# LukasHedegaard/continual-skeletons

Measured on AMD Instinct MI355X. Metric: clips/sec (ST-GCN clip forward, NTU-60 shape; CoST-GCN online step reported under costgcn_online), higher is better.
Workload: dtype f32

## Files before the change

### continual-skeletons_amd/csrc/tcn_wino.hip

```cpp
#include "mfma_core.h"
#include "tcn_params.h"

namespace {

constexpr int WMT = 64;
constexpr int WNT = 128;
constexpr int WTAPS = 12;

template <int VT>
constexpr int wino_ldb() { return ((2 * ((WNT + VT - 2) / VT) + 10) * VT + 3) / 4 * 4; }

struct WStage12x64 {
    unsigned goff0, loff0, gstride;
    f32x4 v[6];
    __device__ __forceinline__ void setup(int Cpad, int Mpad, int tid) {
        goff0 = (unsigned)(((tid >> 7) * Cpad + ((tid >> 4) & 7)) * Mpad + (tid & 15) * 4);
        loff0 = (unsigned)(tid * 4);
        gstride = (unsigned)(2 * Cpad * Mpad);
    }
    __device__ __forceinline__ void issue_slot(int u, const float *__restrict__ chunk_base) {
        v[u] = *reinterpret_cast<const f32x4 *>(chunk_base + (size_t)u * gstride + goff0);
    }
    __device__ __forceinline__ void issue(const float *__restrict__ chunk_base) {
#pragma unroll
        for (int u = 0; u < 6; ++u) issue_slot(u, chunk_base);
    }
    __device__ __forceinline__ void commit(float *__restrict__ Wl) const {
#pragma unroll
        for (int u = 0; u < 6; ++u) *reinterpret_cast<f32x4 *>(Wl + u * (NTHREADS * 4) + loff0) = v[u];
    }
};

template <int VT, int G>
__device__ __forceinline__ void wino_group(const float *__restrict__ Wl, const float *__restrict__ Bl, int off, int l31, int kh,
                                           f32x16 (&acc)[4][2]) {
    constexpr int LDB = wino_ldb<VT>();
    const float *br = Bl + kh * LDB + off + 3 * G * VT;
    const float *wr = Wl + 4 * G * (KC * WMT) + kh * WMT + l31;
#pragma unroll
    for (int s = 0; s < KC / 2; ++s) {
        const float d0 = br[2 * s * LDB], d1 = br[2 * s * LDB + VT], d2 = br[2 * s * LDB + 2 * VT], d3 = br[2 * s * LDB + 3 * VT];
        const float b[4] = {d0 - d2, d1 + d2, d2 - d1, d1 - d3};
#pragma unroll
        for (int i = 0; i < 4; ++i) {
            const float a0 = wr[i * (KC * WMT) + 2 * s * WMT], a1 = wr[i * (KC * WMT) + 2 * s * WMT + 32];
            acc[i][0] = __builtin_amdgcn_mfma_f32_32x32x2f32(a0, b[i], acc[i][0], 0, 0, 0);
            acc[i][1] = __builtin_amdgcn_mfma_f32_32x32x2f32(a1, b[i], acc[i][1], 0, 0, 0);
        }
    }
}

template <int VT, bool RES>
__device__ __forceinline__ void wino_epilogue(const TcnParams &p, const f32x16 (&acc)[4][2], int m0, int q0, int qend, int seg,
                                              int wave, int l31, int kh, int jc, int vc) {
    const int T = p.Tout, TV = T * VT;
    const bool qv = q0 + wave * 32 + l31 < qend;
    const bool odd_ok = 2 * jc + 1 < T;
    const unsigned p0 = (unsigned)(2 * jc * VT + vc);
    const unsigned b0 = 4u * (4u * (unsigned)kh * (unsigned)TV + p0);
    const unsigned b1 = odd_ok ? b0 + 4u * VT : b0;
    const unsigned kh16 = 16u * (unsigned)kh;
    const float *rseg = RES ? p.xres + (int64_t)seg * p.Cout * TV : nullptr;
    float *oseg = p.out + (int64_t)seg * p.Cout * TV;
#pragma unroll
    for (int mi = 0; mi < 2; ++mi) {
        const int rb = m0 + mi * 32;
        float o0[16], o1[16];
#pragma unroll
        for (int g = 0; g < 16; ++g) {
            const int row = rb + (g & 3) + 8 * (g >> 2);
            const float bias = ld_lane(p.bias + row, kh16);
            const float m1 = acc[1][mi][g], m2 = acc[2][mi][g];
            float v0 = acc[0][mi][g] + m1 + m2 + bias;
            float v1 = m1 - m2 - acc[3][mi][g] + bias;
            if (RES) {
                const float *rrow = rseg + (int64_t)row * TV;
                v0 += ld_lane(rrow, b0);
                v1 += ld_lane(rrow, b1);
            }
            if (p.relu) { v0 = relu_nan(v0); v1 = relu_nan(v1); }
            o0[g] = v0;
            o1[g] = v1;
        }
        if (qv) {
#pragma unroll
            for (int g = 0; g < 16; ++g) {
                float *orow = oseg + (int64_t)(rb + (g & 3) + 8 * (g >> 2)) * TV;
                st_lane(orow, b0, o0[g]);
                if (odd_ok) st_lane(orow, b1, o1[g]);
            }
        }
    }
}

}

template <int VT, bool RES = true>
__global__ __launch_bounds__(NTHREADS, 2) void tcn_stage_wino_kernel(const TcnParams p) {
    constexpr int LDB = wino_ldb<VT>();
    constexpr int NJ = (LDB + 63) / 64;
    extern __shared__ __attribute__((aligned(16))) float smem[];
    float *Wl = smem;
    float *Bl = smem + WTAPS * KC * WMT;

    const int tid = threadIdx.x, lane = tid & 63, wave = __builtin_amdgcn_readfirstlane(tid >> 6);
    const int l31 = lane & 31, kh = lane >> 5;
    const unsigned wid = xcd_contiguous_id(blockIdx.x, gridDim.x);
    const int m0 = (int)(wid % p.mtiles) * WMT, q0 = (int)((wid / p.mtiles) % p.qtiles) * WNT;
    const int seg = (int)(wid / (p.mtiles * p.qtiles));
    const int T = p.Tout, TV = T * VT, QP = p.nt;
    const int qend = min(q0 + WNT, QP);
    const int ja = div_magic(q0, p.vmagic), jb = div_magic(qend - 1, p.vmagic);

    const int qc = min(q0 + wave * 32 + l31, qend - 1);
    const int jc = div_magic(qc, p.vmagic), vc = qc - jc * VT;
    const int off = 2 * (jc - ja) * VT + vc;

    f32x16 acc[4][2];
#pragma unroll
    for (int i = 0; i < 4; ++i)
#pragma unroll
        for (int mi = 0; mi < 2; ++mi)
#pragma unroll
            for (int g = 0; g < 16; ++g) acc[i][mi][g] = 0.f;

    {
        const int fa = 2 * ja - 4;
        const int span = (2 * (jb - ja) + 10) * VT;
        const int64_t cs = (int64_t)TV;
        const float *seg_base = p.y + (int64_t)seg * p.C * cs;
        const float *wbase = p.w + m0;
        WStage12x64 ws;
        ws.setup(p.Cpad, p.Mpad, tid);
        auto kloop = [&](auto &bx) {
            ws.issue(wbase);
            bx.issue(seg_base, p.C, cs, 0, wave);
            for (int c0 = 0; c0 + KC < p.Cpad; c0 += KC) {
                __syncthreads();
                ws.commit(Wl);
                bx.commit(Bl, LDB, wave);
                __syncthreads();
                const float *wnext = wbase + (size_t)(c0 + KC) * p.Mpad;
                const int cn = c0 + KC;
                ws.issue_slot(0, wnext);
                ws.issue_slot(1, wnext);
                bx.template issue_third<0>(seg_base, p.C, cs, cn, wave);
                __builtin_amdgcn_s_setprio(1);
                wino_group<VT, 0>(Wl, Bl, off, l31, kh, acc);
                __builtin_amdgcn_s_setprio(0);
                ws.issue_slot(2, wnext);
                ws.issue_slot(3, wnext);
                bx.template issue_third<1>(seg_base, p.C, cs, cn, wave);
                __builtin_amdgcn_s_setprio(1);
                wino_group<VT, 1>(Wl, Bl, off, l31, kh, acc);
                __builtin_amdgcn_s_setprio(0);
                ws.issue_slot(4, wnext);
                ws.issue_slot(5, wnext);
                bx.template issue_third<2>(seg_base, p.C, cs, cn, wave);
                __builtin_amdgcn_s_setprio(1);
                wino_group<VT, 2>(Wl, Bl, off, l31, kh, acc);
                __builtin_amdgcn_s_setprio(0);
            }
            __syncthreads();
            ws.commit(Wl);
            bx.commit(Bl, LDB, wave);
            __syncthreads();
            wino_group<VT, 0>(Wl, Bl, off, l31, kh, acc);
            wino_group<VT, 1>(Wl, Bl, off, l31, kh, acc);
            wino_group<VT, 2>(Wl, Bl, off, l31, kh, acc);
        };
        const bool interior = fa >= 0 && fa * VT + 4 * ((span + 3) / 4) <= TV;
        if (interior) {
            BStage4<(NJ + 3) / 4> b4;
            b4.setup(fa * VT, span, lane);
            kloop(b4);
        } else {
            BStage<NJ> bs;
            bs.setup(fa * VT, span, TV, lane);
            kloop(bs);
        }
    }

    wino_epilogue<VT, RES>(p, acc, m0, q0, qend, seg, wave, l31, kh, jc, vc);
}

namespace {

constexpr int W2TAPS = 13;

template <int VT>
constexpr int wino2_ldb() { return ((4 * ((WNT + VT - 2) / VT) + 11) * VT + 3) / 4 * 4; }

struct WStage13x64 {
    unsigned goff0, loff0, gstride, u6;
    f32x4 v[7];
    __device__ __forceinline__ void setup(int Cpad, int Mpad, int tid) {
        goff0 = (unsigned)(((tid >> 7) * Cpad + ((tid >> 4) & 7)) * Mpad + (tid & 15) * 4);
        loff0 = (unsigned)(tid * 4);
        gstride = (unsigned)(2 * Cpad * Mpad);
        u6 = tid >= 128 ? 5u : 6u;
    }
    __device__ __forceinline__ void issue_slot(int u, const float *__restrict__ chunk_base) {
        if (u < 6) v[u] = *reinterpret_cast<const f32x4 *>(chunk_base + (size_t)u * gstride + goff0);
        else v[6] = *reinterpret_cast<const f32x4 *>(chunk_base + (size_t)u6 * gstride + goff0);
    }
    __device__ __forceinline__ void issue(const float *__restrict__ chunk_base) {
#pragma unroll
        for (int u = 0; u < 7; ++u) issue_slot(u, chunk_base);
    }
    __device__ __forceinline__ void commit(float *__restrict__ Wl) const {
#pragma unroll
        for (int u = 0; u < 6; ++u) *reinterpret_cast<f32x4 *>(Wl + u * (NTHREADS * 4) + loff0) = v[u];
        *reinterpret_cast<f32x4 *>(Wl + u6 * (NTHREADS * 4) + loff0) = v[6];
    }
};

struct WStageRes64 {
    unsigned goff0, loff0;
    f32x4 v;
    __device__ __forceinline__ void setup(int Mpad, int tid) {
        goff0 = (unsigned)(((tid >> 4) & 7) * Mpad + (tid & 15) * 4);
        loff0 = (unsigned)((tid & 127) * 4);
    }
    __device__ __forceinline__ void issue(const float *__restrict__ chunk_base) {
        v = *reinterpret_cast<const f32x4 *>(chunk_base + goff0);
    }
    __device__ __forceinline__ void commit(float *__restrict__ Wl) const { *reinterpret_cast<f32x4 *>(Wl + loff0) = v; }
};

template <int VT, int ROW0, int F, int NP>
__device__ __forceinline__ void wino2_group(const float *__restrict__ Wl, const float *__restrict__ Bl, int off, int l31, int kh,
                                            f32x16 (&acc)[4][2]) {
    constexpr int LDB = wino2_ldb<VT>();
    const float *br = Bl + kh * LDB + off + F * VT;
    const float *wr = Wl + ROW0 * (KC * WMT) + kh * WMT + l31;
#pragma unroll
    for (int s = 0; s < KC / 2; ++s) {
        const float d0 = br[2 * s * LDB], d1 = br[2 * s * LDB + 2 * VT], d2 = br[2 * s * LDB + 4 * VT];
        const float d3 = NP == 4 ? br[2 * s * LDB + 6 * VT] : 0.f;
        const float b[4] = {d0 - d2, d1 + d2, d2 - d1, d1 - d3};
#pragma unroll
        for (int i = 0; i < NP; ++i) {
            const float a0 = wr[i * (KC * WMT) + 2 * s * WMT], a1 = wr[i * (KC * WMT) + 2 * s * WMT + 32];
            acc[i][0] = __builtin_amdgcn_mfma_f32_32x32x2f32(a0, b[i], acc[i][0], 0, 0, 0);
            acc[i][1] = __builtin_amdgcn_mfma_f32_32x32x2f32(a1, b[i], acc[i][1], 0, 0, 0);
        }
    }
}

template <int VT>
__device__ __forceinline__ void wino2_res_chunk(const float *__restrict__ Wl, const float *__restrict__ Bl, int off, int l31, int kh,
                                                f32x16 (&acc)[4][2]) {
    constexpr int LDB = wino2_ldb<VT>();
    const float *br = Bl + kh * LDB + off;
    const float *wr = Wl + kh * WMT + l31;
#pragma unroll
    for (int s = 0; s < KC / 2; ++s) {
        const float d0 = br[2 * s * LDB], d1 = br[2 * s * LDB + 2 * VT];
        const float a0 = wr[2 * s * WMT], a1 = wr[2 * s * WMT + 32];
        const float b0 = d0 - d1;
        acc[0][0] = __builtin_amdgcn_mfma_f32_32x32x2f32(a0, b0, acc[0][0], 0, 0, 0);
        acc[0][1] = __builtin_amdgcn_mfma_f32_32x32x2f32(a1, b0, acc[0][1], 0, 0, 0);
        acc[1][0] = __builtin_amdgcn_mfma_f32_32x32x2f32(a0, d1, acc[1][0], 0, 0, 0);
        acc[1][1] = __builtin_amdgcn_mfma_f32_32x32x2f32(a1, d1, acc[1][1], 0, 0, 0);
    }
}

}

template <int VT, bool RESCONV>
__global__ __launch_bounds__(NTHREADS, 2) void tcn_stage_wino_s2_kernel(const TcnParams p) {
    constexpr int LDB = wino2_ldb<VT>();
    constexpr int NJ = (LDB + 63) / 64;
    constexpr int NJR = ((4 * ((WNT + VT - 2) / VT) + 3) * VT + 63) / 64;
    extern __shared__ __attribute__((aligned(16))) float smem[];
    float *Wl = smem;
    float *Bl = smem + W2TAPS * KC * WMT;

    const int tid = threadIdx.x, lane = tid & 63, wave = __builtin_amdgcn_readfirstlane(tid >> 6);
    const int l31 = lane & 31, kh = lane >> 5;
    const unsigned wid = xcd_contiguous_id(blockIdx.x, gridDim.x);
    const int m0 = (int)(wid % p.mtiles) * WMT, q0 = (int)((wid / p.mtiles) % p.qtiles) * WNT;
    const int seg = (int)(wid / (p.mtiles * p.qtiles));
    const int TVin = p.Tin * VT, QP = p.nt;
    const int qend = min(q0 + WNT, QP);
    const int ja = div_magic(q0, p.vmagic), jb = div_magic(qend - 1, p.vmagic);

    const int qc = min(q0 + wave * 32 + l31, qend - 1);
    const int jc = div_magic(qc, p.vmagic), vc = qc - jc * VT;
    const int off = 4 * (jc - ja) * VT + vc;

    f32x16 acc[4][2];
#pragma unroll
    for (int i = 0; i < 4; ++i)
#pragma unroll
        for (int mi = 0; mi < 2; ++mi)
#pragma unroll
            for (int g = 0; g < 16; ++g) acc[i][mi][g] = 0.f;

    {
        const int fa = 4 * ja - 4;
        const int span = (4 * (jb - ja) + 11) * VT;
        const int64_t cs = (int64_t)TVin;
        const float *seg_base = p.y + (int64_t)seg * p.C * cs;
        const float *wbase = p.w + m0;
        WStage13x64 ws;
        ws.setup(p.Cpad, p.Mpad, tid);
        auto kloop = [&](auto &bx) {
            ws.issue(wbase);
            bx.issue(seg_base, p.C, cs, 0, wave);
            for (int c0 = 0; c0 + KC < p.Cpad; c0 += KC) {
                __syncthreads();
                ws.commit(Wl);
                bx.commit(Bl, LDB, wave);
                __syncthreads();
                const float *wnext = wbase + (size_t)(c0 + KC) * p.Mpad;
                const int cn = c0 + KC;
                ws.issue_slot(0, wnext);
                ws.issue_slot(1, wnext);
                bx.template issue_third<0>(seg_base, p.C, cs, cn, wave);
                __builtin_amdgcn_s_setprio(1);
                wino2_group<VT, 0, 0, 4>(Wl, Bl, off, l31, kh, acc);
                __builtin_amdgcn_s_setprio(0);
                ws.issue_slot(2, wnext);
                ws.issue_slot(3, wnext);
                bx.template issue_third<1>(seg_base, p.C, cs, cn, wave);
                __builtin_amdgcn_s_setprio(1);
                wino2_group<VT, 4, 6, 3>(Wl, Bl, off, l31, kh, acc);
                __builtin_amdgcn_s_setprio(0);
                ws.issue_slot(4, wnext);
                ws.issue_slot(5, wnext);
                bx.template issue_third<2>(seg_base, p.C, cs, cn, wave);
                __builtin_amdgcn_s_setprio(1);
                wino2_group<VT, 7, 1, 3>(Wl, Bl, off, l31, kh, acc);
                __builtin_amdgcn_s_setprio(0);
                ws.issue_slot(6, wnext);
                __builtin_amdgcn_s_setprio(1);
                wino2_group<VT, 10, 5, 3>(Wl, Bl, off, l31, kh, acc);
                __builtin_amdgcn_s_setprio(0);
            }
            __syncthreads();
            ws.commit(Wl);
            bx.commit(Bl, LDB, wave);
            __syncthreads();
            wino2_group<VT, 0, 0, 4>(Wl, Bl, off, l31, kh, acc);
            wino2_group<VT, 4, 6, 3>(Wl, Bl, off, l31, kh, acc);
            wino2_group<VT, 7, 1, 3>(Wl, Bl, off, l31, kh, acc);
            wino2_group<VT, 10, 5, 3>(Wl, Bl, off, l31, kh, acc);
        };
        const bool interior = fa >= 0 && fa * VT + 4 * ((span + 3) / 4) <= TVin;
        if (interior) {
            BStage4<(NJ + 3) / 4> b4;
            b4.setup(fa * VT, span, lane);
            kloop(b4);
        } else {
            BStage<NJ> bs;
            bs.setup(fa * VT, span, TVin, lane);
            kloop(bs);
        }
    }

    if (RESCONV) {
        const int span = (4 * (jb - ja) + 3) * VT;
        const int64_t cs = (int64_t)p.Tres * VT;
        const float *seg_base = p.xres + (int64_t)seg * p.Cres * cs;
        const float *wbase = p.wres + m0;
        const int cend = (p.Cres + KC - 1) / KC * KC;
        WStageRes64 wr;
        wr.setup(p.Mpad, tid);
        BStage<NJR> bs;
        bs.setup(4 * ja * VT, span, p.Tres * VT, lane);
        wr.issue(wbase);
        bs.issue(seg_base, p.Cres, cs, 0, wave);
        for (int c0 = 0; c0 + KC < cend; c0 += KC) {
            __syncthreads();
            wr.commit(Wl);
            bs.commit(Bl, LDB, wave);
            __syncthreads();
            wr.issue(wbase + (size_t)(c0 + KC) * p.Mpad);
            bs.issue(seg_base, p.Cres, cs, c0 + KC, wave);
            wino2_res_chunk<VT>(Wl, Bl, off, l31, kh, acc);
        }
        __syncthreads();
        wr.commit(Wl);
        bs.commit(Bl, LDB, wave);
        __syncthreads();
        wino2_res_chunk<VT>(Wl, Bl, off, l31, kh, acc);
    }

    wino_epilogue<VT, false>(p, acc, m0, q0, qend, seg, wave, l31, kh, jc, vc);
}

static int tcn_stage_wino_launch(const float *y, const float *w_wino, const float *x_res, const float *bias, float *out, int n_seg,
                                 int c, int c_out, int t_in, int V, int k, int stride, int pad, int res_mode, int c_res, int t_res,
                                 int res_off, int relu, void *stream, bool res_none = false) {
    if (!w_wino || !y || !bias || !out) return -2;
    if (k != 9 || stride != 1 || pad != 4) return -2;
    if (res_none ? res_mode != CSK_RES_NONE : (res_mode != CSK_RES_IDENTITY || res_off != 0 || !x_res || c_res != c_out || t_res != t_in))
        return -2;
    if ((V != 25 && V != 18) || c_out % WMT != 0 || c < 1 || n_seg < 1 || t_in < 1) return -2;
    if ((int64_t)t_in * V >= (1 << 26)) return -2;
    if (csk_diag_flag("CSK_TCN_WINO")) return -2;
    const int qp = (t_in + 1) / 2 * V;
    const int qtiles = (qp + WNT - 1) / WNT, mtiles = c_out / WMT;
    if ((int64_t)qtiles * mtiles * n_seg >= (1ll << 31)) return -2;
    TcnParams p = {};
    p.y = y; p.w = w_wino; p.xres = res_none ? nullptr : x_res; p.wres = nullptr; p.bias = bias; p.out = out;
    p.C = c; p.Cpad = round_up(c, CSK_CPAD); p.Cout = c_out; p.Mpad = round_up(c_out, CSK_MT);
    p.Tin = t_in; p.Tout = t_in; p.V = V; p.K = k; p.stride = 1; p.pad = pad;
    p.res_mode = res_mode; p.Cres = res_none ? 0 : c_res; p.CresPad = round_up(p.Cres, CSK_CPAD); p.Tres = res_none ? 0 : t_res;
    p.res_off = 0; p.relu = relu;
    p.vmagic = vmagic_of(V); p.mtiles = (unsigned)mtiles; p.qtiles = (unsigned)qtiles; p.nt = qp;
    void (*kern)(TcnParams) = res_none ? (V == 25 ? tcn_stage_wino_kernel<25, false> : tcn_stage_wino_kernel<18, false>)
                                       : (V == 25 ? tcn_stage_wino_kernel<25> : tcn_stage_wino_kernel<18>);
    const int ldb = V == 25 ? wino_ldb<25>() : wino_ldb<18>();
    p.ldb = ldb;
    const size_t lds = (size_t)(WTAPS * KC * WMT + KC * ldb) * sizeof(float);
    if (const int e = csk_ensure_lds((const void *)kern, lds)) return e;
    hipLaunchKernelGGL(kern, dim3((unsigned)(qtiles * mtiles * n_seg)), dim3(NTHREADS), lds, (hipStream_t)stream, p);
    return (int)hipGetLastError();
}

static int tcn_stage_wino_s2_launch(const float *y, const float *w_s2, const float *x_res, const float *w_res, const float *bias,
                                    float *out, int n_seg, int c, int c_out, int t_in, int V, int k, int stride, int pad,
                                    int res_mode, int c_res, int t_res, int res_off, int relu, void *stream) {
    if (!w_s2 || !y || !bias || !out) return -2;
    if (k != 9 || stride != 2 || pad != 4 || res_off != 0) return -2;
    const bool conv = res_mode == CSK_RES_CONV;
    if (!conv && res_mode != CSK_RES_NONE) return -2;
    if (conv && (!x_res || !w_res || c_res < 1 || t_res != t_in)) return -2;
    if ((V != 25 && V != 18) || c_out % WMT != 0 || c < 1 || n_seg < 1 || t_in < 1) return -2;
    if ((int64_t)t_in * V >= (1 << 26)) return -2;
    if (csk_diag_flag("CSK_TCN_WINO")) return -2;
    const int t_out = (t_in - 1) / 2 + 1;
    const int qp = (t_out + 1) / 2 * V;
    const int qtiles = (qp + WNT - 1) / WNT, mtiles = c_out / WMT;
    if ((int64_t)qtiles * mtiles * n_seg >= (1ll << 31)) return -2;
    TcnParams p = {};
    p.y = y; p.w = w_s2; p.xres = conv ? x_res : nullptr; p.wres = conv ? w_res : nullptr; p.bias = bias; p.out = out;
    p.C = c; p.Cpad = round_up(c, CSK_CPAD); p.Cout = c_out; p.Mpad = round_up(c_out, CSK_MT);
    p.Tin = t_in; p.Tout = t_out; p.V = V; p.K = k; p.stride = 2; p.pad = pad;
    p.res_mode = res_mode; p.Cres = conv ? c_res : 0; p.CresPad = round_up(p.Cres, CSK_CPAD); p.Tres = conv ? t_res : 0;
    p.res_off = 0; p.relu = relu;
    p.vmagic = vmagic_of(V); p.mtiles = (unsigned)mtiles; p.qtiles = (unsigned)qtiles; p.nt = qp;
    void (*kern)(TcnParams) = conv ? (V == 25 ? tcn_stage_wino_s2_kernel<25, true> : tcn_stage_wino_s2_kernel<18, true>)
                                   : (V == 25 ? tcn_stage_wino_s2_kernel<25, false> : tcn_stage_wino_s2_kernel<18, false>);
    const int ldb = V == 25 ? wino2_ldb<25>() : wino2_ldb<18>();
    p.ldb = ldb;
    const size_t lds = (size_t)(W2TAPS * KC * WMT + KC * ldb) * sizeof(float);
    if (const int e = csk_ensure_lds((const void *)kern, lds)) return e;
    hipLaunchKernelGGL(kern, dim3((unsigned)(qtiles * mtiles * n_seg)), dim3(NTHREADS), lds, (hipStream_t)stream, p);
    return (int)hipGetLastError();
}

extern "C" int csk_tcn_stage_wino_f32(const float *y, const float *w, const float *x_res, const float *w_res, const float *bias,
                                      float *out, int n_seg, int c, int c_out, int t_in, int V, int k, int stride, int pad,
                                      int res_mode, int c_res, int t_res, int res_off, int relu, const float *w_wino, void *stream) {
    const int rc = tcn_stage_wino_launch(y, w_wino, x_res, bias, out, n_seg, c, c_out, t_in, V, k, stride, pad, res_mode, c_res,
                                         t_res, res_off, relu, stream);
    if (rc != -2) return rc;
    return csk_tcn_stage_f32(y, w, x_res, w_res, bias, out, n_seg, c, c_out, t_in, V, k, stride, pad, res_mode, c_res, t_res,
                             res_off, relu, stream);
}

extern "C" int csk_tcn_stage_wino_ext_f32(const float *y, const float *w, const float *x_res, const float *w_res, const float *bias,
                                          float *out, int n_seg, int c, int c_out, int t_in, int V, int k, int stride, int pad,
                                          int res_mode, int c_res, int t_res, int res_off, int relu, const float *w_wino_ext,
                                          void *stream) {
    int rc = -2;
    if (stride == 1)
        rc = tcn_stage_wino_launch(y, w_wino_ext, nullptr, bias, out, n_seg, c, c_out, t_in, V, k, stride, pad, res_mode, c_res,
                                   t_res, res_off, relu, stream, true);
    else if (stride == 2)
        rc = tcn_stage_wino_s2_launch(y, w_wino_ext, x_res, w_res, bias, out, n_seg, c, c_out, t_in, V, k, stride, pad, res_mode,
                                      c_res, t_res, res_off, relu, stream);
    if (rc != -2) return rc;
    return csk_tcn_stage_f32(y, w, x_res, w_res, bias, out, n_seg, c, c_out, t_in, V, k, stride, pad, res_mode, c_res, t_res,
                             res_off, relu, stream);
}
```

Before: 4158.

## Add 128x64 Winograd TCN tile variant with 2x2 wave layout

Adds an MW=2 variant of the stride-1 and stride-2 Winograd temporal-conv kernels. Each block covers 128 output channels by 64 positions, with waves arranged 2x2 instead of 1x4, and new weight and input staging structs sized for the taller tile. A heuristic uses it by default for stride-2 stages, and for stride-1 stages when the narrower position tile wastes less padding. The aim is more reuse of the input B-tile across output channels and less tail waste on the position axis. The cost is a larger LDS weight footprint, fewer blocks in flight, and more template instantiations.

Result: faster. 4268 (median of 6 runs) (+2.7%).

```diff
diff --git a/continual-skeletons_amd/csrc/tcn_wino.hip b/continual-skeletons_amd/csrc/tcn_wino.hip
--- a/continual-skeletons_amd/csrc/tcn_wino.hip
+++ b/continual-skeletons_amd/csrc/tcn_wino.hip
@@ -1,3 +1,5 @@
+#include <type_traits>
+
 #include "mfma_core.h"
 #include "tcn_params.h"
 
@@ -7,8 +9,8 @@
 constexpr int WNT = 128;
 constexpr int WTAPS = 12;
 
-template <int VT>
-constexpr int wino_ldb() { return ((2 * ((WNT + VT - 2) / VT) + 10) * VT + 3) / 4 * 4; }
+template <int VT, int MW = 1>
+constexpr int wino_ldb() { return ((2 * ((WNT / MW + VT - 2) / VT) + 10) * VT + 3) / 4 * 4; }
 
 struct WStage12x64 {
     unsigned goff0, loff0, gstride;
@@ -25,25 +27,58 @@
 #pragma unroll
         for (int u = 0; u < 6; ++u) issue_slot(u, chunk_base);
     }
+    template <int G>
+    __device__ __forceinline__ void issue_part(const float *__restrict__ chunk_base) {
+        issue_slot(2 * G, chunk_base);
+        issue_slot(2 * G + 1, chunk_base);
+    }
     __device__ __forceinline__ void commit(float *__restrict__ Wl) const {
 #pragma unroll
         for (int u = 0; u < 6; ++u) *reinterpret_cast<f32x4 *>(Wl + u * (NTHREADS * 4) + loff0) = v[u];
     }
 };
 
-template <int VT, int G>
+template <int NT>
+struct WStageNx128 {
+    unsigned goff0, loff0, gstride;
+    f32x4 v[NT];
+    __device__ __forceinline__ void setup(int Cpad, int Mpad, int tid) {
+        goff0 = 4u * (unsigned)((tid >> 5) * Mpad + (tid & 31) * 4);
+        loff0 = (unsigned)(tid * 4);
+        gstride = (unsigned)(Cpad * Mpad);
+    }
+    __device__ __forceinline__ void issue_slot(int u, const float *__restrict__ chunk_base) {
+        v[u] = *reinterpret_cast<const f32x4 *>(reinterpret_cast<const char *>(chunk_base + (size_t)u * gstride) + goff0);
+    }
+    __device__ __forceinline__ void issue(const float *__restrict__ chunk_base) {
+#pragma unroll
+        for (int u = 0; u < NT; ++u) issue_slot(u, chunk_base);
+    }
+    template <int G>
+    __device__ __forceinline__ void issue_part(const float *__restrict__ chunk_base) {
+        constexpr int lo = NT == 13 ? (G == 0 ? 0 : 3 * G + 1) : 4 * G, hi = NT == 13 ? 3 * G + 4 : 4 * G + 4;
+#pragma unroll
+        for (int u = lo; u < hi; ++u) issue_slot(u, chunk_base);
+    }
+    __device__ __forceinline__ void commit(float *__restrict__ Wl) const {
+#pragma unroll
+        for (int u = 0; u < NT; ++u) *reinterpret_cast<f32x4 *>(Wl + u * (KC * 128) + loff0) = v[u];
+    }
+};
+
+template <int VT, int G, int MW>
 __device__ __forceinline__ void wino_group(const float *__restrict__ Wl, const float *__restrict__ Bl, int off, int l31, int kh,
                                            f32x16 (&acc)[4][2]) {
-    constexpr int LDB = wino_ldb<VT>();
+    constexpr int LDB = wino_ldb<VT, MW>(), MT = WMT * MW;
     const float *br = Bl + kh * LDB + off + 3 * G * VT;
-    const float *wr = Wl + 4 * G * (KC * WMT) + kh * WMT + l31;
+    const float *wr = Wl + 4 * G * (KC * MT) + kh * MT + l31;
 #pragma unroll
     for (int s = 0; s < KC / 2; ++s) {
         const float d0 = br[2 * s * LDB], d1 = br[2 * s * LDB + VT], d2 = br[2 * s * LDB + 2 * VT], d3 = br[2 * s * LDB + 3 * VT];
         const float b[4] = {d0 - d2, d1 + d2, d2 - d1, d1 - d3};
 #pragma unroll
         for (int i = 0; i < 4; ++i) {
-            const float a0 = wr[i * (KC * WMT) + 2 * s * WMT], a1 = wr[i * (KC * WMT) + 2 * s * WMT + 32];
+            const float a0 = wr[i * (KC * MT) + 2 * s * MT], a1 = wr[i * (KC * MT) + 2 * s * MT + 32];
             acc[i][0] = __builtin_amdgcn_mfma_f32_32x32x2f32(a0, b[i], acc[i][0], 0, 0, 0);
             acc[i][1] = __builtin_amdgcn_mfma_f32_32x32x2f32(a1, b[i], acc[i][1], 0, 0, 0);
         }
@@ -52,9 +87,9 @@
 
 template <int VT, bool RES>
 __device__ __forceinline__ void wino_epilogue(const TcnParams &p, const f32x16 (&acc)[4][2], int m0, int q0, int qend, int seg,
-                                              int wave, int l31, int kh, int jc, int vc) {
+                                              int wn, int l31, int kh, int jc, int vc) {
     const int T = p.Tout, TV = T * VT;
-    const bool qv = q0 + wave * 32 + l31 < qend;
+    const bool qv = q0 + wn * 32 + l31 < qend;
     const bool odd_ok = 2 * jc + 1 < T;
     const unsigned p0 = (unsigned)(2 * jc * VT + vc);
     const unsigned b0 = 4u * (4u * (unsigned)kh * (unsigned)TV + p0);
@@ -95,24 +130,25 @@
 
 }
 
-template <int VT, bool RES = true>
+template <int VT, bool RES = true, int MW = 1>
 __global__ __launch_bounds__(NTHREADS, 2) void tcn_stage_wino_kernel(const TcnParams p) {
-    constexpr int LDB = wino_ldb<VT>();
+    constexpr int LDB = wino_ldb<VT, MW>(), MT = WMT * MW, NT = WNT / MW;
     constexpr int NJ = (LDB + 63) / 64;
     extern __shared__ __attribute__((aligned(16))) float smem[];
     float *Wl = smem;
-    float *Bl = smem + WTAPS * KC * WMT;
+    float *Bl = smem + WTAPS * KC * MT;
 
     const int tid = threadIdx.x, lane = tid & 63, wave = __builtin_amdgcn_readfirstlane(tid >> 6);
     const int l31 = lane & 31, kh = lane >> 5;
+    const int wm = MW == 2 ? wave >> 1 : 0, wn = MW == 2 ? wave & 1 : wave;
     const unsigned wid = xcd_contiguous_id(blockIdx.x, gridDim.x);
-    const int m0 = (int)(wid % p.mtiles) * WMT, q0 = (int)((wid / p.mtiles) % p.qtiles) * WNT;
+    const int m0 = (int)(wid % p.mtiles) * MT, q0 = (int)((wid / p.mtiles) % p.qtiles) * NT;
     const int seg = (int)(wid / (p.mtiles * p.qtiles));
     const int T = p.Tout, TV = T * VT, QP = p.nt;
-    const int qend = min(q0 + WNT, QP);
+    const int qend = min(q0 + NT, QP);
     const int ja = div_magic(q0, p.vmagic), jb = div_magic(qend - 1, p.vmagic);
 
-    const int qc = min(q0 + wave * 32 + l31, qend - 1);
+    const int qc = min(q0 + wn * 32 + l31, qend - 1);
     const int jc = div_magic(qc, p.vmagic), vc = qc - jc * VT;
     const int off = 2 * (jc - ja) * VT + vc;
 
@@ -130,7 +166,8 @@
         const int64_t cs = (int64_t)TV;
         const float *seg_base = p.y + (int64_t)seg * p.C * cs;
         const float *wbase = p.w + m0;
-        WStage12x64 ws;
+        const float *Ww = Wl + wm * WMT;
+        std::conditional_t<MW == 2, WStageNx128<WTAPS>, WStage12x64> ws;
         ws.setup(p.Cpad, p.Mpad, tid);
         auto kloop = [&](auto &bx) {
             ws.issue(wbase);
@@ -142,32 +179,29 @@
                 __syncthreads();
                 const float *wnext = wbase + (size_t)(c0 + KC) * p.Mpad;
                 const int cn = c0 + KC;
-                ws.issue_slot(0, wnext);
-                ws.issue_slot(1, wnext);
+                ws.template issue_part<0>(wnext);
                 bx.template issue_third<0>(seg_base, p.C, cs, cn, wave);
                 __builtin_amdgcn_s_setprio(1);
-                wino_group<VT, 0>(Wl, Bl, off, l31, kh, acc);
+                wino_group<VT, 0, MW>(Ww, Bl, off, l31, kh, acc);
                 __builtin_amdgcn_s_setprio(0);
-                ws.issue_slot(2, wnext);
-                ws.issue_slot(3, wnext);
+                ws.template issue_part<1>(wnext);
                 bx.template issue_third<1>(seg_base, p.C, cs, cn, wave);
                 __builtin_amdgcn_s_setprio(1);
-                wino_group<VT, 1>(Wl, Bl, off, l31, kh, acc);
+                wino_group<VT, 1, MW>(Ww, Bl, off, l31, kh, acc);
                 __builtin_amdgcn_s_setprio(0);
-                ws.issue_slot(4, wnext);
-                ws.issue_slot(5, wnext);
+                ws.template issue_part<2>(wnext);
                 bx.template issue_third<2>(seg_base, p.C, cs, cn, wave);
                 __builtin_amdgcn_s_setprio(1);
-                wino_group<VT, 2>(Wl, Bl, off, l31, kh, acc);
+                wino_group<VT, 2, MW>(Ww, Bl, off, l31, kh, acc);
                 __builtin_amdgcn_s_setprio(0);
             }
             __syncthreads();
             ws.commit(Wl);
             bx.commit(Bl, LDB, wave);
             __syncthreads();
-            wino_group<VT, 0>(Wl, Bl, off, l31, kh, acc);
-            wino_group<VT, 1>(Wl, Bl, off, l31, kh, acc);
-            wino_group<VT, 2>(Wl, Bl, off, l31, kh, acc);
+            wino_group<VT, 0, MW>(Ww, Bl, off, l31, kh, acc);
+            wino_group<VT, 1, MW>(Ww, Bl, off, l31, kh, acc);
+            wino_group<VT, 2, MW>(Ww, Bl, off, l31, kh, acc);
         };
         const bool interior = fa >= 0 && fa * VT + 4 * ((span + 3) / 4) <= TV;
         if (interior) {
@@ -181,15 +215,15 @@
         }
     }
 
-    wino_epilogue<VT, RES>(p, acc, m0, q0, qend, seg, wave, l31, kh, jc, vc);
+    wino_epilogue<VT, RES>(p, acc, m0 + wm * WMT, q0, qend, seg, wn, l31, kh, jc, vc);
 }
 
 namespace {
 
 constexpr int W2TAPS = 13;
 
-template <int VT>
-constexpr int wino2_ldb() { return ((4 * ((WNT + VT - 2) / VT) + 11) * VT + 3) / 4 * 4; }
+template <int VT, int MW = 1>
+constexpr int wino2_ldb() { return ((4 * ((WNT / MW + VT - 2) / VT) + 11) * VT + 3) / 4 * 4; }
 
 struct WStage13x64 {
     unsigned goff0, loff0, gstride, u6;
@@ -208,6 +242,15 @@
 #pragma unroll
         for (int u = 0; u < 7; ++u) issue_slot(u, chunk_base);
     }
+    template <int G>
+    __device__ __forceinline__ void issue_part(const float *__restrict__ chunk_base) {
+        if (G < 3) {
+            issue_slot(2 * G, chunk_base);
+            issue_slot(2 * G + 1, chunk_base);
+        } else {
+            issue_slot(6, chunk_base);
+        }
+    }
     __device__ __forceinline__ void commit(float *__restrict__ Wl) const {
 #pragma unroll
         for (int u = 0; u < 6; ++u) *reinterpret_cast<f32x4 *>(Wl + u * (NTHREADS * 4) + loff0) = v[u];
@@ -228,12 +271,77 @@
     __device__ __forceinline__ void commit(float *__restrict__ Wl) const { *reinterpret_cast<f32x4 *>(Wl + loff0) = v; }
 };
 
-template <int VT, int ROW0, int F, int NP>
+struct WStageRes128 {
+    unsigned goff0, loff0;
+    f32x4 v;
+    __device__ __forceinline__ void setup(int Mpad, int tid) {
+        goff0 = (unsigned)((tid >> 5) * Mpad + (tid & 31) * 4);
+        loff0 = (unsigned)(tid * 4);
+    }
+    __device__ __forceinline__ void issue(const float *__restrict__ chunk_base) {
+        v = *reinterpret_cast<const f32x4 *>(chunk_base + goff0);
+    }
+    __device__ __forceinline__ void commit(float *__restrict__ Wl) const { *reinterpret_cast<f32x4 *>(Wl + loff0) = v; }
+};
+
+template <int LDB>
+struct BStage4Tail {
+    static constexpr int RPW = KC / (NTHREADS / 64);
+    static constexpr int REST = LDB % 256;
+    static constexpr int NV = LDB / 256 + (REST > 128 ? 1 : 0), NS = REST > 128 ? 0 : (REST + 63) / 64;
+    static_assert(NV >= 1 && NV <= 2 && NS <= 2, "issue_third: 16-byte sweeps with thirds 0 and 1, 4-byte sweeps with third 2");
+    unsigned off4[NV], off1[NS > 0 ? NS : 1];
+    int pbase_;
+    f32x4 v[RPW][NV];
+    float t[RPW][NS > 0 ? NS : 1];
+    __device__ __forceinline__ void setup(int pbase, int span, int lane) {
+        const int nvec = (span + 3) / 4;
+        pbase_ = pbase;
+#pragma unroll
+        for (int u = 0; u < NV; ++u) off4[u] = (unsigned)(4 * min(u * 64 + lane, nvec - 1));
+#pragma unroll
+        for (int u = 0; u < NS; ++u) off1[u] = (unsigned)min(NV * 256 + u * 64 + lane, span - 1);
+    }
+    __device__ __forceinline__ const float *row(const float *__restrict__ seg_base, int C, int64_t chan_stride, int c0, int wave,
+                                                int rr) const {
+        const int c = min(c0 + wave + rr * (NTHREADS / 64), C - 1);
+        return seg_base + (int64_t)c * chan_stride + pbase_;
+    }
+    template <int G>
+    __device__ __forceinline__ void issue_third(const float *__restrict__ seg_base, int C, int64_t chan_stride, int c0, int wave) {
+#pragma unroll
+        for (int rr = 0; rr < RPW; ++rr) {
+            const float *src = row(seg_base, C, chan_stride, c0, wave, rr);
+            if (G < NV) v[rr][G < NV ? G : 0] = *reinterpret_cast<const f32x4u *>(src + off4[G < NV ? G : 0]);
+            if (G == 2) {
+#pragma unroll
+                for (int u = 0; u < NS; ++u) t[rr][u] = src[off1[u]];
+            }
+        }
+    }
+    __device__ __forceinline__ void issue(const float *__restrict__ seg_base, int C, int64_t chan_stride, int c0, int wave) {
+        issue_third<0>(seg_base, C, chan_stride, c0, wave);
+        issue_third<1>(seg_base, C, chan_stride, c0, wave);
+        issue_third<2>(seg_base, C, chan_stride, c0, wave);
+    }
+    __device__ __forceinline__ void commit(float *__restrict__ Bl, int ldb, int wave) const {
+#pragma unroll
+        for (int rr = 0; rr < RPW; ++rr) {
+            float *dst = Bl + (wave + rr * (NTHREADS / 64)) * ldb;
+#pragma unroll
+            for (int u = 0; u < NV; ++u) *reinterpret_cast<f32x4 *>(dst + off4[u]) = v[rr][u];
+#pragma unroll
+            for (int u = 0; u < NS; ++u) dst[off1[u]] = t[rr][u];
+        }
+    }
+};
+
+template <int VT, int ROW0, int F, int NP, int MW>
 __device__ __forceinline__ void wino2_group(const float *__restrict__ Wl, const float *__restrict__ Bl, int off, int l31, int kh,
                                             f32x16 (&acc)[4][2]) {
-    constexpr int LDB = wino2_ldb<VT>();
+    constexpr int LDB = wino2_ldb<VT, MW>(), MT = WMT * MW;
     const float *br = Bl + kh * LDB + off + F * VT;
-    const float *wr = Wl + ROW0 * (KC * WMT) + kh * WMT + l31;
+    const float *wr = Wl + ROW0 * (KC * MT) + kh * MT + l31;
 #pragma unroll
     for (int s = 0; s < KC / 2; ++s) {
         const float d0 = br[2 * s * LDB], d1 = br[2 * s * LDB + 2 * VT], d2 = br[2 * s * LDB + 4 * VT];
@@ -241,23 +349,23 @@
         const float b[4] = {d0 - d2, d1 + d2, d2 - d1, d1 - d3};
 #pragma unroll
         for (int i = 0; i < NP; ++i) {
-            const float a0 = wr[i * (KC * WMT) + 2 * s * WMT], a1 = wr[i * (KC * WMT) + 2 * s * WMT + 32];
+            const float a0 = wr[i * (KC * MT) + 2 * s * MT], a1 = wr[i * (KC * MT) + 2 * s * MT + 32];
             acc[i][0] = __builtin_amdgcn_mfma_f32_32x32x2f32(a0, b[i], acc[i][0], 0, 0, 0);
             acc[i][1] = __builtin_amdgcn_mfma_f32_32x32x2f32(a1, b[i], acc[i][1], 0, 0, 0);
         }
     }
 }
 
-template <int VT>
+template <int VT, int MW>
 __device__ __forceinline__ void wino2_res_chunk(const float *__restrict__ Wl, const float *__restrict__ Bl, int off, int l31, int kh,
                                                 f32x16 (&acc)[4][2]) {
-    constexpr int LDB = wino2_ldb<VT>();
+    constexpr int LDB = wino2_ldb<VT, MW>(), MT = WMT * MW;
     const float *br = Bl + kh * LDB + off;
-    const float *wr = Wl + kh * WMT + l31;
+    const float *wr = Wl + kh * MT + l31;
 #pragma unroll
     for (int s = 0; s < KC / 2; ++s) {
         const float d0 = br[2 * s * LDB], d1 = br[2 * s * LDB + 2 * VT];
-        const float a0 = wr[2 * s * WMT], a1 = wr[2 * s * WMT + 32];
+        const float a0 = wr[2 * s * MT], a1 = wr[2 * s * MT + 32];
         const float b0 = d0 - d1;
         acc[0][0] = __builtin_amdgcn_mfma_f32_32x32x2f32(a0, b0, acc[0][0], 0, 0, 0);
         acc[0][1] = __builtin_amdgcn_mfma_f32_32x32x2f32(a1, b0, acc[0][1], 0, 0, 0);
@@ -268,25 +376,27 @@
 
 }
 
-template <int VT, bool RESCONV>
+template <int VT, bool RESCONV, int MW = 1>
 __global__ __launch_bounds__(NTHREADS, 2) void tcn_stage_wino_s2_kernel(const TcnParams p) {
-    constexpr int LDB = wino2_ldb<VT>();
+    constexpr int LDB = wino2_ldb<VT, MW>(), MT = WMT * MW, NT = WNT / MW;
     constexpr int NJ = (LDB + 63) / 64;
-    constexpr int NJR = ((4 * ((WNT + VT - 2) / VT) + 3) * VT + 63) / 64;
+    constexpr int NJR = ((4 * ((NT + VT - 2) / VT) + 3) * VT + 63) / 64;
     extern __shared__ __attribute__((aligned(16))) float smem[];
     float *Wl = smem;
-    float *Bl = smem + W2TAPS * KC * WMT;
+    float *Bl = smem + W2TAPS * KC * MT;
 
     const int tid = threadIdx.x, lane = tid & 63, wave = __builtin_amdgcn_readfirstlane(tid >> 6);
     const int l31 = lane & 31, kh = lane >> 5;
+    const int wm = MW == 2 ? wave >> 1 : 0, wn = MW == 2 ? wave & 1 : wave;
     const unsigned wid = xcd_contiguous_id(blockIdx.x, gridDim.x);
-    const int m0 = (int)(wid % p.mtiles) * WMT, q0 = (int)((wid / p.mtiles) % p.qtiles) * WNT;
+    const int m0 = (int)(wid % p.mtiles) * MT, q0 = (int)((wid / p.mtiles) % p.qtiles) * NT;
     const int seg = (int)(wid / (p.mtiles * p.qtiles));
     const int TVin = p.Tin * VT, QP = p.nt;
-    const int qend = min(q0 + WNT, QP);
+    const int qend = min(q0 + NT, QP);
     const int ja = div_magic(q0, p.vmagic), jb = div_magic(qend - 1, p.vmagic);
-
-    const int qc = min(q0 + wave * 32 + l31, qend - 1);
+    const float *Ww = Wl + wm * WMT;
+
+    const int qc = min(q0 + wn * 32 + l31, qend - 1);
     const int jc = div_magic(qc, p.vmagic), vc = qc - jc * VT;
     const int off = 4 * (jc - ja) * VT + vc;
 
@@ -304,7 +414,7 @@
         const int64_t cs = (int64_t)TVin;
         const float *seg_base = p.y + (int64_t)seg * p.C * cs;
         const float *wbase = p.w + m0;
-        WStage13x64 ws;
+        std::conditional_t<MW == 2, WStageNx128<W2TAPS>, WStage13x64> ws;
         ws.setup(p.Cpad, p.Mpad, tid);
         auto kloop = [&](auto &bx) {
             ws.issue(wbase);
@@ -316,41 +426,38 @@
                 __syncthreads();
                 const float *wnext = wbase + (size_t)(c0 + KC) * p.Mpad;
                 const int cn = c0 + KC;
-                ws.issue_slot(0, wnext);
-                ws.issue_slot(1, wnext);
+                ws.template issue_part<0>(wnext);
                 bx.template issue_third<0>(seg_base, p.C, cs, cn, wave);
                 __builtin_amdgcn_s_setprio(1);
-                wino2_group<VT, 0, 0, 4>(Wl, Bl, off, l31, kh, acc);
+                wino2_group<VT, 0, 0, 4, MW>(Ww, Bl, off, l31, kh, acc);
                 __builtin_amdgcn_s_setprio(0);
-                ws.issue_slot(2, wnext);
-                ws.issue_slot(3, wnext);
+                ws.template issue_part<1>(wnext);
                 bx.template issue_third<1>(seg_base, p.C, cs, cn, wave);
                 __builtin_amdgcn_s_setprio(1);
-                wino2_group<VT, 4, 6, 3>(Wl, Bl, off, l31, kh, acc);
+                wino2_group<VT, 4, 6, 3, MW>(Ww, Bl, off, l31, kh, acc);
                 __builtin_amdgcn_s_setprio(0);
-                ws.issue_slot(4, wnext);
-                ws.issue_slot(5, wnext);
+                ws.template issue_part<2>(wnext);
                 bx.template issue_third<2>(seg_base, p.C, cs, cn, wave);
                 __builtin_amdgcn_s_setprio(1);
-                wino2_group<VT, 7, 1, 3>(Wl, Bl, off, l31, kh, acc);
+                wino2_group<VT, 7, 1, 3, MW>(Ww, Bl, off, l31, kh, acc);
                 __builtin_amdgcn_s_setprio(0);
-                ws.issue_slot(6, wnext);
+                ws.template issue_part<3>(wnext);
                 __builtin_amdgcn_s_setprio(1);
-                wino2_group<VT, 10, 5, 3>(Wl, Bl, off, l31, kh, acc);
+                wino2_group<VT, 10, 5, 3, MW>(Ww, Bl, off, l31, kh, acc);
                 __builtin_amdgcn_s_setprio(0);
             }
             __syncthreads();
             ws.commit(Wl);
             bx.commit(Bl, LDB, wave);
             __syncthreads();
-            wino2_group<VT, 0, 0, 4>(Wl, Bl, off, l31, kh, acc);
-            wino2_group<VT, 4, 6, 3>(Wl, Bl, off, l31, kh, acc);
-            wino2_group<VT, 7, 1, 3>(Wl, Bl, off, l31, kh, acc);
-            wino2_group<VT, 10, 5, 3>(Wl, Bl, off, l31, kh, acc);
+            wino2_group<VT, 0, 0, 4, MW>(Ww, Bl, off, l31, kh, acc);
+            wino2_group<VT, 4, 6, 3, MW>(Ww, Bl, off, l31, kh, acc);
+            wino2_group<VT, 7, 1, 3, MW>(Ww, Bl, off, l31, kh, acc);
+            wino2_group<VT, 10, 5, 3, MW>(Ww, Bl, off, l31, kh, acc);
         };
         const bool interior = fa >= 0 && fa * VT + 4 * ((span + 3) / 4) <= TVin;
         if (interior) {
-            BStage4<(NJ + 3) / 4> b4;
+            std::conditional_t<MW == 2, BStage4Tail<LDB>, BStage4<(NJ + 3) / 4>> b4;
             b4.setup(fa * VT, span, lane);
             kloop(b4);
         } else {
@@ -366,7 +473,7 @@
         const float *seg_base = p.xres + (int64_t)seg * p.Cres * cs;
         const float *wbase = p.wres + m0;
         const int cend = (p.Cres + KC - 1) / KC * KC;
-        WStageRes64 wr;
+        std::conditional_t<MW == 2, WStageRes128, WStageRes64> wr;
         wr.setup(p.Mpad, tid);
         BStage<NJR> bs;
         bs.setup(4 * ja * VT, span, p.Tres * VT, lane);
@@ -379,16 +486,25 @@
             __syncthreads();
             wr.issue(wbase + (size_t)(c0 + KC) * p.Mpad);
             bs.issue(seg_base, p.Cres, cs, c0 + KC, wave);
-            wino2_res_chunk<VT>(Wl, Bl, off, l31, kh, acc);
+            wino2_res_chunk<VT, MW>(Ww, Bl, off, l31, kh, acc);
         }
         __syncthreads();
         wr.commit(Wl);
         bs.commit(Bl, LDB, wave);
         __syncthreads();
-        wino2_res_chunk<VT>(Wl, Bl, off, l31, kh, acc);
-    }
-
-    wino_epilogue<VT, false>(p, acc, m0, q0, qend, seg, wave, l31, kh, jc, vc);
+        wino2_res_chunk<VT, MW>(Ww, Bl, off, l31, kh, acc);
+    }
+
+    wino_epilogue<VT, false>(p, acc, m0 + wm * WMT, q0, qend, seg, wn, l31, kh, jc, vc);
+}
+
+static int wino_pick_mw(int qp, int c_out, int stride) {
+    if (c_out % (2 * WMT) != 0) return 1;
+    const int force = csk_diag_int("CSK_TCN_WINO");
+    if (force == 2 || force == 3) return force - 1;
+    if (stride == 2) return 2;
+    const int64_t wide = round_up(qp, WNT), tall = round_up(qp, WNT / 2);
+    return 16 * tall <= 15 * wide ? 2 : 1;
 }
 
 static int tcn_stage_wino_launch(const float *y, const float *w_wino, const float *x_res, const float *bias, float *out, int n_seg,
@@ -400,9 +516,10 @@
         return -2;
     if ((V != 25 && V != 18) || c_out % WMT != 0 || c < 1 || n_seg < 1 || t_in < 1) return -2;
     if ((int64_t)t_in * V >= (1 << 26)) return -2;
-    if (csk_diag_flag("CSK_TCN_WINO")) return -2;
+    if (csk_diag_flag("CSK_TCN_WINO") && csk_diag_int("CSK_TCN_WINO") < 2) return -2;
     const int qp = (t_in + 1) / 2 * V;
-    const int qtiles = (qp + WNT - 1) / WNT, mtiles = c_out / WMT;
+    const int mw = wino_pick_mw(qp, c_out, stride);
+    const int qtiles = (qp + WNT / mw - 1) / (WNT / mw), mtiles = c_out / (WMT * mw);
     if ((int64_t)qtiles * mtiles * n_seg >= (1ll << 31)) return -2;
     TcnParams p = {};
     p.y = y; p.w = w_wino; p.xres = res_none ? nullptr : x_res; p.wres = nullptr; p.bias = bias; p.out = out;
@@ -411,11 +528,19 @@
     p.res_mode = res_mode; p.Cres = res_none ? 0 : c_res; p.CresPad = round_up(p.Cres, CSK_CPAD); p.Tres = res_none ? 0 : t_res;
     p.res_off = 0; p.relu = relu;
     p.vmagic = vmagic_of(V); p.mtiles = (unsigned)mtiles; p.qtiles = (unsigned)qtiles; p.nt = qp;
-    void (*kern)(TcnParams) = res_none ? (V == 25 ? tcn_stage_wino_kernel<25, false> : tcn_stage_wino_kernel<18, false>)
-                                       : (V == 25 ? tcn_stage_wino_kernel<25> : tcn_stage_wino_kernel<18>);
-    const int ldb = V == 25 ? wino_ldb<25>() : wino_ldb<18>();
+    void (*kern)(TcnParams);
+    int ldb;
+    if (mw == 2) {
+        kern = res_none ? (V == 25 ? tcn_stage_wino_kernel<25, false, 2> : tcn_stage_wino_kernel<18, false, 2>)
+                        : (V == 25 ? tcn_stage_wino_kernel<25, true, 2> : tcn_stage_wino_kernel<18, true, 2>);
+        ldb = V == 25 ? wino_ldb<25, 2>() : wino_ldb<18, 2>();
+    } else {
+        kern = res_none ? (V == 25 ? tcn_stage_wino_kernel<25, false> : tcn_stage_wino_kernel<18, false>)
+                        : (V == 25 ? tcn_stage_wino_kernel<25> : tcn_stage_wino_kernel<18>);
+        ldb = V == 25 ? wino_ldb<25>() : wino_ldb<18>();
+    }
     p.ldb = ldb;
-    const size_t lds = (size_t)(WTAPS * KC * WMT + KC * ldb) * sizeof(float);
+    const size_t lds = (size_t)(WTAPS * KC * WMT * mw + KC * ldb) * sizeof(float);
     if (const int e = csk_ensure_lds((const void *)kern, lds)) return e;
     hipLaunchKernelGGL(kern, dim3((unsigned)(qtiles * mtiles * n_seg)), dim3(NTHREADS), lds, (hipStream_t)stream, p);
     return (int)hipGetLastError();
@@ -431,10 +556,11 @@
     if (conv && (!x_res || !w_res || c_res < 1 || t_res != t_in)) return -2;
     if ((V != 25 && V != 18) || c_out % WMT != 0 || c < 1 || n_seg < 1 || t_in < 1) return -2;
     if ((int64_t)t_in * V >= (1 << 26)) return -2;
-    if (csk_diag_flag("CSK_TCN_WINO")) return -2;
+    if (csk_diag_flag("CSK_TCN_WINO") && csk_diag_int("CSK_TCN_WINO") < 2) return -2;
     const int t_out = (t_in - 1) / 2 + 1;
     const int qp = (t_out + 1) / 2 * V;
-    const int qtiles = (qp + WNT - 1) / WNT, mtiles = c_out / WMT;
+    const int mw = wino_pick_mw(qp, c_out, stride);
+    const int qtiles = (qp + WNT / mw - 1) / (WNT / mw), mtiles = c_out / (WMT * mw);
     if ((int64_t)qtiles * mtiles * n_seg >= (1ll << 31)) return -2;
     TcnParams p = {};
     p.y = y; p.w = w_s2; p.xres = conv ? x_res : nullptr; p.wres = conv ? w_res : nullptr; p.bias = bias; p.out = out;
@@ -443,11 +569,19 @@
     p.res_mode = res_mode; p.Cres = conv ? c_res : 0; p.CresPad = round_up(p.Cres, CSK_CPAD); p.Tres = conv ? t_res : 0;
     p.res_off = 0; p.relu = relu;
     p.vmagic = vmagic_of(V); p.mtiles = (unsigned)mtiles; p.qtiles = (unsigned)qtiles; p.nt = qp;
-    void (*kern)(TcnParams) = conv ? (V == 25 ? tcn_stage_wino_s2_kernel<25, true> : tcn_stage_wino_s2_kernel<18, true>)
-                                   : (V == 25 ? tcn_stage_wino_s2_kernel<25, false> : tcn_stage_wino_s2_kernel<18, false>);
-    const int ldb = V == 25 ? wino2_ldb<25>() : wino2_ldb<18>();
+    void (*kern)(TcnParams);
+    int ldb;
+    if (mw == 2) {
+        kern = conv ? (V == 25 ? tcn_stage_wino_s2_kernel<25, true, 2> : tcn_stage_wino_s2_kernel<18, true, 2>)
+                    : (V == 25 ? tcn_stage_wino_s2_kernel<25, false, 2> : tcn_stage_wino_s2_kernel<18, false, 2>);
+        ldb = V == 25 ? wino2_ldb<25, 2>() : wino2_ldb<18, 2>();
+    } else {
+        kern = conv ? (V == 25 ? tcn_stage_wino_s2_kernel<25, true> : tcn_stage_wino_s2_kernel<18, true>)
+                    : (V == 25 ? tcn_stage_wino_s2_kernel<25, false> : tcn_stage_wino_s2_kernel<18, false>);
+        ldb = V == 25 ? wino2_ldb<25>() : wino2_ldb<18>();
+    }
     p.ldb = ldb;
-    const size_t lds = (size_t)(W2TAPS * KC * WMT + KC * ldb) * sizeof(float);
+    const size_t lds = (size_t)(W2TAPS * KC * WMT * mw + KC * ldb) * sizeof(float);
     if (const int e = csk_ensure_lds((const void *)kern, lds)) return e;
     hipLaunchKernelGGL(kern, dim3((unsigned)(qtiles * mtiles * n_seg)), dim3(NTHREADS), lds, (hipStream_t)stream, p);
     return (int)hipGetLastError();
```
